# drapado/PINGS

Hardware: AMD Instinct MI355X
Metric: raster fwd+bwd Mpix/s @1M Gaussians 1080p (higher is better)
Workload: dtype f32; 1 GPU; surfel rasteriser fwd+bwd, 1000000 Gaussians, 1920x1080, one view per GPU; gaussians=1000000, width=1920, height=1080

## Files before the change

include/pings_hip.h:

```cpp
#ifndef PINGS_HIP_H_
#define PINGS_HIP_H_

#include <stddef.h>
#include <stdint.h>

#if defined(__cplusplus)
#define PINGS_EXTERN_C extern "C"
#else
#define PINGS_EXTERN_C
#endif
#define PINGS_API PINGS_EXTERN_C __attribute__((visibility("default")))

#define PINGS_OK 0
#define PINGS_ERR_ARG 1
#define PINGS_ERR_HIP 2
#define PINGS_ERR_CAPACITY 3


#define PINGS_ABI_VERSION 11
PINGS_API int pings_abi_version(void);
PINGS_API const char* pings_last_error(void);

PINGS_API int pings_prof_enable(int on);
PINGS_API int pings_prof_only(const char* stage);
// ... 69 lines not shown

PINGS_API int pings_raster_backward(const pings_raster_settings* s, int P, int64_t num_instances,
                                    const float* means3D, const float* colors,
                                    const float* opacities, const float* scales,
                                    const float* rotations, const void* geom_blob,
                                    const void* binning_blob, const void* image_blob,
                                    const float* out_color, const float* out_normal,
                                    const float* out_depth, const float* out_alpha,
                                    const float* dL_dcolor, const float* dL_dnormal,
                                    const float* dL_ddepth, const float* dL_dalpha,
                                    void* bwd_blob, float* dL_dmeans3D, float* dL_dmeans2D,
                                    float* dL_dcolors, float* dL_dopacities, float* dL_dscales,
                                    float* dL_drotations, float* dL_dtau, int footprint_class,
                                    void* stream);

PINGS_API int pings_raster_debug_lists(const void* binning_blob, int64_t num_instances,
                                       int image_height, int image_width, uint32_t* point_list,
                                       uint32_t* ranges_xy, void* stream);
PINGS_API int pings_raster_debug_image(const void* image_blob, int image_height, int image_width,
                                       float* final_T, uint32_t* n_contrib, void* stream);
PINGS_API int pings_raster_debug_occlusion(const void* geom_blob, int P, int image_height, int image_width,
                                           uint32_t* occ_bucket, uint16_t* occ_bsat, int32_t* occ_nb,
                                           void* stream);


PINGS_API size_t pings_raster2d_geom_bytes(int P, int image_height, int image_width);
PINGS_API size_t pings_raster2d_binning_bytes(int64_t num_instances, int image_height, int image_width);
PINGS_API size_t pings_raster2d_image_bytes(int image_height, int image_width);

PINGS_API int pings_raster2d_preprocess(const pings_raster_settings* s, int P, const float* means3D,
                                        const float* colors, const float* opacities, const float* scales,
                                        const float* rotations, void* geom_blob, int32_t* radii,
                                        const int32_t* live_rows_dev, int dyn_rows, const int32_t* const* aux_dev,
                                        int aux_words, int32_t* aux_host, int64_t* num_instances, void* stream);

PINGS_API int pings_raster2d_render(const pings_raster_settings* s, int P, int64_t num_instances, void* geom_blob,
                                    void* binning_blob, void* image_blob, float* out_color, float* out_allmap,
                                    void* stream);

PINGS_API size_t pings_raster2d_backward_bytes(int P, int64_t num_instances);

PINGS_API int pings_raster2d_backward(const pings_raster_settings* s, int P, int64_t num_instances,
                                      const float* scales, const float* rotations, const void* geom_blob,
                                      const void* binning_blob, const void* image_blob, const float* dL_dcolor,
                                      const float* dL_dallmap, void* bwd_blob, float* dL_dmeans3D,
                                      float* dL_dmeans2D, float* dL_dcolors, float* dL_dopacities,
// ... 714 lines not shown
```

pings_amd/_abi.py:

```python
from __future__ import annotations

import ctypes as C

ABI_VERSION = 11

RASTER_SURFEL, RASTER_3DGS, RASTER_2DGS = 0, 1, 2
HEAD_COLOR, HEAD_SEMANTIC = 0, 1
REG_SINGULAR, REG_ILL_CONDITIONED, REG_NONFINITE = 1, 2, 4
REG_F_NORMALS, REG_F_DIV_GRAD, REG_F_WEIGHTED = 1, 2, 4
REG_COLOR_PHOTO, REG_COLOR_CONSIST = 1, 2
MC_ALLOW_DEGENERATE, MC_ASCENT = 1, 2
ADAMW_MAX_JOBS, ADAMW_CHUNK = 48, 4096
EVAL_VIEW_RECORD, EVAL_PAIR_RECORD = 9, 12
EVAL_EXTENT = 1
LOOP_MAX_R, LOOP_MAX_S, LOOP_MAX_D = 32, 128, 16
LOOP_MAX_Q, LOOP_MAX_C = 16, 65536
LIDAR_MAX_CAMS, LIDAR_MAX_LIDARS = 8, 8
TSDF_BLOCK = 8
TSDF_EXTENT, TSDF_TABLE_FULL = 1, 2

vp = C.c_void_p
i32, i64, f32, f64, sz = C.c_int, C.c_int64, C.c_float, C.c_double, C.c_size_t


# ... 152 lines not shown
    "pings_prof_report": (i32, [C.c_char_p, sz]),
    "pings_ssim_partials_count": (sz, [i32, i32, i32]),
    "pings_ssim_forward": (i32, [vp, vp, i32, i32, i32, i32, vp, vp, vp, vp, vp, vp]),
    "pings_ssim_backward": (i32, [vp, vp, i32, i32, i32, vp, vp, vp, vp, vp, vp]),
    "pings_raster_mark_visible": (i32, [vp, i32, C.POINTER(RasterSettings), vp, vp]),
    "pings_raster_geom_bytes": (sz, [i32, i32, i32]),
    "pings_raster_binning_bytes": (sz, [i64, i32, i32]),
    "pings_raster_image_bytes": (sz, [i32, i32]),
    "pings_raster_preprocess": (i32, [C.POINTER(RasterSettings), i32, vp, vp, vp, vp, vp, vp, vp, C.POINTER(i64),
                                      C.POINTER(i32), vp]),
    "pings_raster_preprocess_dyn": (i32, [C.POINTER(RasterSettings), i32, vp, vp, vp, vp, vp, vp, vp, vp, i32,
                                          C.POINTER(vp), i32, C.POINTER(i32), C.POINTER(i64), C.POINTER(i32), vp]),
    "pings_raster_render": (i32, [C.POINTER(RasterSettings), i32, i64, vp, vp, vp, vp, vp, vp, vp, vp, i32, vp]),
    "pings_raster_tile_sort_bytes": (sz, [i64, C.POINTER(i32)]),
    "pings_raster_tile_sort": (i32, [vp, i64, i32, i32, vp, vp, vp, i32, vp]),
    "pings_raster_scan_bytes": (sz, [i64]),
    "pings_raster_scan_u32": (i32, [vp, i64, i32, i32, vp, vp, sz, vp]),
    "pings_raster_backward_bytes": (sz, [i32, i64]),
    "pings_raster_backward": (i32, [C.POINTER(RasterSettings), i32, i64, vp, vp, vp, vp, vp, vp, vp, vp, vp, vp, vp, vp,
                                    vp, vp, vp, vp, vp, vp, vp, vp, vp, vp, vp, vp, i32, vp]),
    "pings_raster_debug_lists": (i32, [vp, i64, i32, i32, vp, vp, vp]),
    "pings_raster_debug_image": (i32, [vp, i32, i32, vp, vp, vp]),
    "pings_raster_debug_occlusion": (i32, [vp, i32, i32, i32, vp, vp, C.POINTER(C.c_int32), vp]),
    "pings_raster2d_geom_bytes": (sz, [i32, i32, i32]),
    "pings_raster2d_binning_bytes": (sz, [i64, i32, i32]),
    "pings_raster2d_image_bytes": (sz, [i32, i32]),
    "pings_raster2d_preprocess": (i32, [C.POINTER(RasterSettings), i32, vp, vp, vp, vp, vp, vp, vp, vp, i32,
                                        C.POINTER(vp), i32, C.POINTER(i32), C.POINTER(i64), vp]),
    "pings_raster2d_render": (i32, [C.POINTER(RasterSettings), i32, i64, vp, vp, vp, vp, vp, vp]),
    "pings_raster2d_backward_bytes": (sz, [i32, i64]),
    "pings_raster2d_backward": (i32, [C.POINTER(RasterSettings), i32, i64, vp, vp, vp, vp, vp, vp, vp, vp, vp, vp, vp,
                                      vp, vp, vp, vp]),
    "pings_raster2d_debug_lists": (i32, [vp, i64, i32, i32, vp, vp, vp]),
    "pings_raster2d_debug_image": (i32, [vp, i32, i32, vp, vp, vp, vp]),
    "pings_knn_compact_entries": (sz, [i64]),
    "pings_knn_compact_build": (i32, [vp, i64, vp, sz, vp]),
    "pings_knn_blocks_entries": (sz, [i64]),
    "pings_knn_blocks_build": (i32, [C.POINTER(KnnMap), i64, i64, i32, vp, sz, vp, vp, vp]),
    "pings_knn_search": (i32, [C.POINTER(KnnMap), vp, i64, vp, vp, vp, vp, vp]),
    "pings_knn_cells": (i32, [C.POINTER(KnnMap), vp, i64, i64, vp, vp, vp]),
    "pings_query_feature_forward": (i32, [C.POINTER(KnnMap), C.POINTER(QfTables), vp, i64, vp, vp, vp, vp, vp, vp, vp,
                                          vp, vp, vp, vp, vp]),
    "pings_query_feature_accumulate": (i32, [vp, vp, i64, vp, vp]),
    "pings_query_feature_scratch_bytes": (sz, [i64, i32, i64]),
    "pings_query_feature_backward": (i32, [C.POINTER(QfTables), vp, vp, i64, i32, vp, vp, vp, vp, vp, vp, i64, vp, vp,
                                           vp, vp, vp]),
# ... 163 lines not shown
```

pings_amd/csrc/raster_blend_fwd.hip:

```cpp
#include "raster_common.hpp"

namespace pings {
namespace raster {

template <int MODE>
__device__ __forceinline__ void blend_fwd_wave_body(
    const KParams& p, const uint2* __restrict__ ranges, const uint32_t* __restrict__ point_list,
    const float4* __restrict__ rec, const uint32_t* __restrict__ gval, float* __restrict__ out_color,
    float* __restrict__ out_normal, float* __restrict__ out_depth, float* __restrict__ out_alpha,
    float* __restrict__ final_T, uint32_t* __restrict__ n_contrib, float* __restrict__ inst_wq,
    uint32_t* __restrict__ inst_cntq, const uint32_t* __restrict__ tile_order,
    const uint32_t* __restrict__ seg_tile_unit0, const unsigned block) {
  __shared__ float4 sA_[4][64], sB_[4][64], sC_[4][64], sD_[4][64];
  __shared__ uint32_t sSlot_[4][64];
  __shared__ int sE_[4][64];
  __shared__ float sW_[4][64];
  __shared__ uint32_t sCnt_[4][64];

  const int lane = threadIdx.x & 63, q = (int)(threadIdx.x >> 6);
  float4 *sA = sA_[q], *sB = sB_[q], *sC = sC_[q], *sD = sD_[q];
  uint32_t *sSlot = sSlot_[q], *sCnt = sCnt_[q];
  int* sE = sE_[q];
  float* sW = sW_[q];
  const int tile = (int)tile_order[block];
// ... 754 lines not shown
  if (MODE == MODE_3DGS) {
    const uint4 c = cq[i];
    inst_cnt[i] = c.x + c.y + c.z + c.w;
  }
}

__device__ inline uint32_t wave_reduce_sum_u32(uint32_t v) {
#pragma unroll
  for (int off = 32; off > 0; off >>= 1) v += (uint32_t)__shfl_xor((int)v, off, 64);
  return v;
}

constexpr int SMALL_RUN = 16;
template <typename T>
__global__ __launch_bounds__(256) void per_gaussian_sum_kernel(
    int P, const uint32_t* __restrict__ gidx_sorted, const uint32_t* __restrict__ nvalid,
    const uint32_t* __restrict__ offsets_sorted, const uint32_t* __restrict__ tiles_sorted,
    const T* __restrict__ inst, T* __restrict__ out) {
  const int r = strided_rank(P);
  const int lane = threadIdx.x & 63;
  uint32_t n = 0, base = 0;
  if (r >= 0 && (uint32_t)r < *nvalid) {
    n = tiles_sorted[r];
    base = offsets_sorted[r] - n;
  }
  T sum = (T)0;
  if (n <= (uint32_t)SMALL_RUN)
    for (uint32_t k = 0; k < n; ++k) sum += inst[base + k];
  unsigned long long m = __ballot(n > (uint32_t)SMALL_RUN);
  while (m) {
    const int src = __ffsll((long long)m) - 1;
    m &= m - 1;
    const uint32_t nb = lane_value(n, src);
    const uint32_t bb = lane_value(base, src);
    T acc = (T)0, acc1 = (T)0, acc2 = (T)0, acc3 = (T)0;
    uint32_t k = lane;
    for (; k + 192 < nb; k += 256) {
      acc += inst[bb + k];
      acc1 += inst[bb + k + 64];
      acc2 += inst[bb + k + 128];
      acc3 += inst[bb + k + 192];
    }
    for (; k < nb; k += 64) acc += inst[bb + k];
    acc = (acc + acc1) + (acc2 + acc3);
    if constexpr (sizeof(T) == 4 && !std::is_integral<T>::value) {
      acc = wave_sum_to_all(acc);
    } else {
      acc = (T)wave_reduce_sum_u32((uint32_t)acc);
    }
    if (lane == src) sum = acc;
  }
  if (r >= 0) out[gidx_sorted[r]] = sum;
}

struct FwdOut {
  float *color, *normal, *depth, *alpha;
};

template <int MODE>
static int launch_blend_fwd_wave(const KParams& kp, const BlendPlan& plan, int64_t I, int num_tiles, const GeomState& gs,
                          const BinState& bs, const ImageState& im, const FwdOut& o, hipStream_t st) {
  const uint32_t seg = plan.seg;
  if (I > 0) PINGS_HIP_CHECK(hipMemsetAsync(bs.inst_wq, 0, 16 * (size_t)I, st));
  if (I > 0 && MODE == MODE_3DGS) PINGS_HIP_CHECK(hipMemsetAsync(bs.inst_cntq, 0, 16 * (size_t)I, st));
  if (!plan.seg_on) {
    hipLaunchKernelGGL((blend_fwd_wave_kernel<MODE>), dim3(num_tiles), dim3(256), 0, st, kp, bs.ranges,
                       bs.point_list, gs.rec, bs.gval, o.color, o.normal, o.depth, o.alpha,
                       im.final_T, im.n_contrib, bs.inst_wq, bs.inst_cntq, bs.tile_order,
                       (const uint32_t*)nullptr);
  } else {
    hipLaunchKernelGGL(seg_plan_kernel, dim3(1), dim3(1024), 0, st, bs.ranges, num_tiles, 2u * seg, seg,
                       bs.seg_max_units, bs.seg_head, bs.seg_unit_tile, bs.seg_unit_seg, bs.seg_tile_unit0);
    PINGS_LAUNCH_CHECK();
    const dim3 gseg(bs.seg_max_units);
    uint16_t* const rel = plan.seg_reuse ? bs.seg_rel : nullptr;
// ... 72 lines not shown
```

pings_amd/csrc/raster_common.hpp:

```cpp
#pragma once
#include <cstdlib>
#include <type_traits>

#include "common.hpp"

namespace pings {
namespace raster {

constexpr int TILE = 16;
constexpr int BLOCK = TILE * TILE;
constexpr float NEAR_Z = 0.2f;
constexpr float LOWPASS = 0.3f;
constexpr float ALPHA_MAX = 0.99f;
constexpr float ALPHA_MIN = 1.0f / 255.0f;
constexpr float T_EPS = 1e-4f;
constexpr float DEPTH_ALPHA_EPS = 1e-10f;
constexpr float DEN_EPS = 1e-6f;
constexpr uint32_t CULLED_KEY = 0xFFFFFFFFu;
constexpr int DS_NB = 1 << 20;
constexpr uint32_t DS_LIMIT = 4096u;
constexpr int DS_SHARDS = 64;
constexpr int DS_KMIN = 2 * DS_SHARDS, DS_SHIFT = DS_KMIN + 1, DS_FLAG = DS_KMIN + 2, DS_HEAD = DS_KMIN + 8;
constexpr float OCC_THR = 9.5f;
constexpr float OCC_FIX = 4096.f;
constexpr uint16_t OCC_ALL = 0xFFFFu;

constexpr int MODE_SURFEL = 0;
constexpr int MODE_3DGS = 1;
constexpr int RECT_TIGHT = 0, RECT_3SIGMA = 1, RECT_ELLIPSE = 2;

constexpr int GRAD_ROW = 16;
constexpr int CH = 64;
enum GradSlot {
  G_MX = 0, G_MY = 1, G_CONX = 2, G_CONY = 3, G_CONZ = 4, G_OPAC = 5,
  G_R = 6, G_G = 7, G_B = 8, G_NX = 9, G_NY = 10, G_NZ = 11, G_Q = 12, G_PZ = 13,
  G_ZLO = 14, G_ZHI = 15
};

struct FrameSummary {
  uint32_t overflow, pad0;
  unsigned long long stats[3];
  int32_t aux[8];
  uint32_t seq;
  uint32_t pad;
};
// ... 165 lines not shown
int tile_sort_library(const KeyT* keys_in, int64_t n, int bits, KeyT* keys_out, uint32_t* vals_out, void* temp,
                      size_t temp_bytes, hipStream_t st);

int launch_blend_fwd(int mode, const KParams& kp, const BlendPlan& plan, int P, int64_t I, const GeomState& gs,
                     const BinState& bs, const ImageState& im, float* out_color, float* out_normal, float* out_depth,
                     float* out_alpha, void* per_gaussian, hipStream_t st);

__device__ inline int lane_value(int v, int src) { return __builtin_amdgcn_readlane(v, src); }
__device__ inline uint32_t lane_value(uint32_t v, int src) { return (uint32_t)__builtin_amdgcn_readlane((int)v, src); }
__device__ inline float lane_value(float v, int src) {
  return __builtin_bit_cast(float, __builtin_amdgcn_readlane(__builtin_bit_cast(int, v), src));
}

__device__ inline int dealt_rank(int num_waves, int wave, int lane) {
  return lane < 16 ? lane * num_waves + wave : ((lane >> 4) * num_waves + wave) * 16 + (lane & 15);
}
__device__ inline int strided_rank(int P) {
  const int num_waves = (int)(gridDim.x * (blockDim.x >> 6));
  const int wave = (int)(blockIdx.x * (blockDim.x >> 6) + (threadIdx.x >> 6));
  const int r = dealt_rank(num_waves, wave, (int)(threadIdx.x & 63));
  return r < P ? r : -1;
}

typedef float f2 __attribute__((ext_vector_type(2)));
__device__ inline f2 f2s(float x) { return f2{x, x}; }
__device__ inline f2 fma2(f2 a, f2 b, f2 c) { return __builtin_elementwise_fma(a, b, c); }
__device__ inline f2 sel2(bool c0, bool c1, f2 a, f2 b) { return f2{c0 ? a.x : b.x, c1 ? a.y : b.y}; }

typedef unsigned long long lmask;
struct cmask {
  unsigned long long bits;
};
enum { LM_OGT = 2, LM_OGE = 3, LM_OLT = 4, LM_OLE = 5 };
__device__ inline cmask mask_lt(float a, float b) { return cmask{__builtin_amdgcn_fcmpf(a, b, LM_OLT)}; }
__device__ inline cmask mask_le(float a, float b) { return cmask{__builtin_amdgcn_fcmpf(a, b, LM_OLE)}; }
__device__ inline cmask mask_gt(float a, float b) { return cmask{__builtin_amdgcn_fcmpf(a, b, LM_OGT)}; }
__device__ inline cmask mask_ge(float a, float b) { return cmask{__builtin_amdgcn_fcmpf(a, b, LM_OGE)}; }
__device__ inline lmask operator&(cmask a, cmask b) { return a.bits & b.bits; }
__device__ inline lmask operator&(lmask a, cmask b) { return a & b.bits; }
__device__ inline lmask operator&(cmask a, lmask b) { return a.bits & b; }
__device__ inline lmask operator|(cmask a, cmask b) { return a.bits | b.bits; }
__device__ inline lmask operator~(cmask a) { return ~a.bits; }
__device__ inline int mask_count(lmask m) { return __builtin_popcountll(m); }
__device__ inline float mask_sel(lmask m, float a, float b) {
  float r;
  asm("v_cndmask_b32_e64 %0, %1, %2, %3" : "=v"(r) : "v"(b), "v"(a), "s"(m));
// ... 293 lines not shown
```

pings_amd/csrc/raster_fwd.hip:

```cpp
#include <hipcub/hipcub.hpp>

#include <algorithm>
#include <chrono>
#include <type_traits>

#include "raster_common.hpp"

namespace pings {
namespace raster {

__device__ inline void to_camera(const float* __restrict__ V, float x, float y, float z, float& px,
                                 float& py, float& pz) {
  px = ((V[0] * x + V[4] * y) + V[8] * z) + V[12];
  py = ((V[1] * x + V[5] * y) + V[9] * z) + V[13];
  pz = ((V[2] * x + V[6] * y) + V[10] * z) + V[14];
}

__global__ __launch_bounds__(256) void mark_visible_kernel(const float* __restrict__ pos, int N,
                                                            const float* __restrict__ V,
                                                            const float* __restrict__ Pm,
                                                            uint8_t* __restrict__ present, int depth_only) {
  const int i = blockIdx.x * blockDim.x + threadIdx.x;
  if (i >= N) return;
  float px, py, pz;
  to_camera(V, pos[3 * i], pos[3 * i + 1], pos[3 * i + 2], px, py, pz);
  const float hx = ((Pm[0] * px + Pm[4] * py) + Pm[8] * pz) + Pm[12];
  const float hy = ((Pm[1] * px + Pm[5] * py) + Pm[9] * pz) + Pm[13];
  const float hw = ((Pm[3] * px + Pm[7] * py) + Pm[11] * pz) + Pm[15];
  const float pw = 1.0f / (hw + 1e-7f);
  const float nx = hx * pw, ny = hy * pw;
  present[i] = (pz > NEAR_Z) && (depth_only || ((nx >= -1.3f) && (nx <= 1.3f) && (ny >= -1.3f) && (ny <= 1.3f)));
}

template <int MODE>
__device__ inline uint32_t preprocess_gaussian(
    const KParams& p, int g, const float* __restrict__ means3D, const float* __restrict__ colors,
    const float* __restrict__ opacities, const float* __restrict__ scales,
    const float* __restrict__ rotations, float4* __restrict__ rec, uint4* __restrict__ rect,
    uint32_t* __restrict__ depth_key, uint32_t* __restrict__ gidx, int32_t* __restrict__ radii) {
  const float* V = p.view;
  const float* Pm = p.proj_raw;

  gidx[g] = (uint32_t)g;
  uint32_t key = CULLED_KEY;
  uint4 rc = make_uint4(0u, 0u, 0u, 0u);
  int rad = 0;

  float px, py, pz;
  to_camera(V, means3D[3 * g], means3D[3 * g + 1], means3D[3 * g + 2], px, py, pz);
  bool ok = pz > NEAR_Z;
  if (p.live && g < p.dyn_rows && g >= *p.live) ok = false;

  const float hx = ((Pm[0] * px + Pm[4] * py) + Pm[8] * pz) + Pm[12];
  const float hy = ((Pm[1] * px + Pm[5] * py) + Pm[9] * pz) + Pm[13];
  const float hw = ((Pm[3] * px + Pm[7] * py) + Pm[11] * pz) + Pm[15];
  const float pw = 1.0f / (hw + 1e-7f);
  const float ndx = hx * pw, ndy = hy * pw;
  const float mx = ((ndx + 1.0f) * (float)p.W - 1.0f) * 0.5f;
  const float my = ((ndy + 1.0f) * (float)p.H - 1.0f) * 0.5f;

  const float qr = rotations[4 * g], qx = rotations[4 * g + 1], qy = rotations[4 * g + 2],
              qz = rotations[4 * g + 3];
// ... 95 lines not shown
        const float thr_u = 2.0f * logf(opac / p.occ_amin);
        const float lam_min = mid - sqrtf(fmaxf(mid * mid - det, 0.0f));
        uint32_t inner = 0xFFFFFFFFu;
        if (thr_u * lam_min >= 50.0f) {
          const float exu = sqrtf(thr_u * cxx), eyu = sqrtf(thr_u * cyy);
          const int ix0 = max(xmin, (int)ceilf((mx - exu) / (float)TILE - 0.02f));
          const int ix1 = min(xmax, (int)floorf((mx + exu - 15.0f) / (float)TILE + 0.02f) + 1);
          const int iy0 = max(ymin, (int)ceilf((my - eyu) / (float)TILE - 0.02f));
          const int iy1 = min(ymax, (int)floorf((my + eyu - 15.0f) / (float)TILE + 0.02f) + 1);
          if (ix1 > ix0 && iy1 > iy0)
            inner = (uint32_t)min(ix0 - xmin, 255) | ((uint32_t)min(xmax - ix1, 255) << 8) |
                    ((uint32_t)min(iy0 - ymin, 255) << 16) | ((uint32_t)min(ymax - iy1, 255) << 24);
        }
        const uint32_t covers = inner;
        rc = make_uint4(covers, (uint32_t)xmin | ((uint32_t)ymin << 16),
                        (uint32_t)xmax | ((uint32_t)ymax << 16), (uint32_t)tiles);
        rad = (int)radius;
      }
    }
  }
  depth_key[g] = key;
  rect[g] = rc;
  radii[g] = rad;
  if (key != CULLED_KEY) {
    rec[4 * g + 0] = make_float4(mx, my, opac, pz);
    rec[4 * g + 1] = make_float4(conic_x, conic_y, conic_z, rz);
    rec[4 * g + 2] = make_float4(colors[3 * g], colors[3 * g + 1], colors[3 * g + 2], q);
    rec[4 * g + 3] = make_float4(nx, ny, nz, 0.0f);
  }
  return key;
}

template <int MODE>
__global__ __launch_bounds__(256) void preprocess_kernel(
    KParams p, const float* __restrict__ means3D, const float* __restrict__ colors,
    const float* __restrict__ opacities, const float* __restrict__ scales,
    const float* __restrict__ rotations, float4* __restrict__ rec, uint4* __restrict__ rect,
    uint32_t* __restrict__ depth_key, uint32_t* __restrict__ gidx, int32_t* __restrict__ radii,
    uint32_t* __restrict__ ds_head) {
  __shared__ uint32_t sm[8];
  const int g = blockIdx.x * blockDim.x + threadIdx.x;
  uint32_t key = CULLED_KEY;
  if (g < p.P)
    key = preprocess_gaussian<MODE>(p, g, means3D, colors, opacities, scales, rotations, rec, rect, depth_key, gidx, radii);
  if (!ds_head) return;
  uint32_t mx = key != CULLED_KEY ? key : 0u, mn = key != CULLED_KEY ? ~key : 0u;
#pragma unroll
  for (int o = 32; o > 0; o >>= 1) {
    mx = max(mx, (uint32_t)__shfl_xor((int)mx, o, 64));
    mn = max(mn, (uint32_t)__shfl_xor((int)mn, o, 64));
  }
  const int wave = threadIdx.x >> 6;
  if ((threadIdx.x & 63) == 0) { sm[wave] = mx; sm[4 + wave] = mn; }
  __syncthreads();
  if (threadIdx.x == 0) {
    mx = max(max(sm[0], sm[1]), max(sm[2], sm[3]));
    mn = max(max(sm[4], sm[5]), max(sm[6], sm[7]));
    if (mx | mn) {
      atomicMax(&ds_head[blockIdx.x % DS_SHARDS], mx);
      atomicMax(&ds_head[DS_SHARDS + blockIdx.x % DS_SHARDS], mn);
    }
  }
}

constexpr int SMALL_RECT = 8;
constexpr int STAT_SHARDS = 256;

struct RectLane {
  uint32_t g, n;
  int xmin, ymin, wdt, hgt;
};
template <typename Serial, typename CoopBegin, typename Coop>
__device__ inline void walk_rects(const RectLane& me, int gx, Serial serial, CoopBegin coop_begin, Coop coop) {
  const int lane = threadIdx.x & 63;
  if (me.n != 0u && me.n <= (uint32_t)SMALL_RECT) {
    int x = 0, y = 0;
    for (uint32_t k = 0; k < me.n; ++k) {
      serial(me.xmin + x, me.ymin + y);
      if (++x == me.wdt) { x = 0; ++y; }
    }
  }
  unsigned long long m = __ballot(me.n > (uint32_t)SMALL_RECT);
  while (m) {
    const int src = __ffsll((long long)m) - 1;
    m &= m - 1;
    const uint32_t n = lane_value(me.n, src);
    const int x0 = lane_value(me.xmin, src), y0 = lane_value(me.ymin, src), wdt = lane_value(me.wdt, src);
    const float inv_w = 1.0f / (float)wdt;
    coop_begin(src);
// ... 247 lines not shown
                                                           uint32_t* __restrict__ rank_of) {
  const int r = blockIdx.x * 256 + threadIdx.x;
  if (r < P) rank_of[gidx_sorted[r]] = (uint32_t)r;
}

__global__ __launch_bounds__(64) void count_valid_kernel(int P, const uint32_t* __restrict__ depth_key_sorted,
                                                         uint32_t* __restrict__ nvalid) {
  const int lane = threadIdx.x;
  long long lo = 0, hi = P;
  while (lo < hi) {
    const long long span = hi - lo;
    const long long step = (span + 63) / 64;
    const long long pos = lo + (long long)lane * step;
    const bool valid = pos < hi && depth_key_sorted[pos] < CULLED_KEY;
    const int nv = __popcll(__ballot(valid));
    if (nv == 0) { hi = lo; break; }
    const long long last_valid = lo + (long long)(nv - 1) * step;
    lo = last_valid + 1;
    hi = min(hi, last_valid + step);
  }
  if (lane == 0) *nvalid = (uint32_t)lo;
}

__device__ inline uint32_t rank_bucket(int r, int nb, uint32_t nvalid) {
  if (r < 0 || nvalid == 0u) return 0u;
  const uint32_t b = (uint32_t)(((unsigned long long)r * (unsigned long long)nb) / (unsigned long long)nvalid);
  return min(b, (uint32_t)nb - 1u);
}

template <bool DENSE>
__global__ __launch_bounds__(256) void occl_budget_kernel(int P, int gx, int nb,
                                                          const uint32_t* __restrict__ gidx_sorted,
                                                          const uint4* __restrict__ rect,
                                                          const float4* __restrict__ rec,
                                                          const uint32_t* __restrict__ nvalid, int num_tiles,
                                                          uint32_t* __restrict__ bucket) {
  const int r = strided_rank(P);
  const uint32_t nv = *nvalid;
  RectLane me = rect_lane(r, gidx_sorted, rect, nv);
  if (me.n != 0u) {
    const uint4 rc = rect[me.g];
    const int x0 = me.xmin + (int)(rc.x & 255u), x1 = (int)(rc.z & 0xFFFF) - (int)((rc.x >> 8) & 255u);
    const int y0 = me.ymin + (int)((rc.x >> 16) & 255u), y1 = (int)(rc.z >> 16) - (int)(rc.x >> 24);
    if (x1 > x0 && y1 > y0) {
      me.xmin = x0; me.ymin = y0; me.wdt = x1 - x0; me.hgt = y1 - y0; me.n = (uint32_t)((x1 - x0) * (y1 - y0));
    } else {
      me.n = 0u;
    }
  }
  float4 ra = make_float4(0.f, 0.f, 0.f, 0.f), rb = ra;
  if (me.n != 0u) {
// ... 103 lines not shown
  __syncthreads();
  const uint32_t sat = tile < num_tiles ? sSat[t] : 0u;
  if (g == 0) {
    uint32_t m = min(sat, (uint32_t)nb - 1u);
#pragma unroll
    for (int o = 32; o > 0; o >>= 1) m = max(m, (uint32_t)__shfl_xor((int)m, o, 64));
    if (t == 0) atomicMax(bmax, m);
  }
  unsigned long long word = 0ull;
  for (int u = 0; u < per; ++u) {
    const unsigned long long w = __ballot(tile < num_tiles && (uint32_t)(g * per + u) <= sat);
    if (t == u) word = w;
  }
  if (t < per) mask[(size_t)(g * per + t) * gridDim.x + blockIdx.x] = word;
}

__global__ __launch_bounds__(256) void count_kept_kernel(int P, int gx, int nb, int words,
                                                         const uint32_t* __restrict__ gidx_sorted,
                                                         const uint4* __restrict__ rect,
                                                         const unsigned long long* __restrict__ mask,
                                                         const uint32_t* __restrict__ nvalid,
                                                         const uint32_t* __restrict__ bmax,
                                                         uint32_t* __restrict__ tiles_sorted,
                                                         unsigned long long* __restrict__ pairs_full) {
  const int r = strided_rank(P);
  const int lane = threadIdx.x & 63;
  const uint32_t nv = *nvalid;
  const RectLane me = rect_lane(r, gidx_sorted, rect, nv);
  const uint32_t bk = rank_bucket(r, nb, nv);
  const uint32_t items = bk <= *bmax ? rect_items(me) : 0u;
  uint32_t kept = 0, acc = 0;
  if (items != 0u && items <= (uint32_t)SMALL_ITEMS)
    walk_items_serial(me, items, gx, mask + (size_t)bk * words,
                      [&](int, unsigned long long bits) { kept += (uint32_t)__popcll(bits); });
  int cur = -1;
  auto flush = [&]() {
    if (cur < 0) return;
#pragma unroll
    for (int off = 32; off > 0; off >>= 1) acc += (uint32_t)__shfl_xor((int)acc, off, 64);
    if (lane == cur) kept = acc;
  };
  walk_items_coop(
      __ballot(items > (uint32_t)SMALL_ITEMS), me, items, gx, bk, mask, words,
      [&](int src) { flush(); cur = src; acc = 0; },
      [&](int, unsigned long long bits) { acc += (uint32_t)__popcll(bits); });
  flush();
  if (r >= 0) tiles_sorted[r] = kept;
  uint32_t tot = me.n;
#pragma unroll
  for (int off = 32; off > 0; off >>= 1) tot += (uint32_t)__shfl_xor((int)tot, off, 64);
  const unsigned long long vis = __ballot(me.n != 0u);
  uint32_t kept_w = r >= 0 ? kept : 0u;
#pragma unroll
  for (int off = 32; off > 0; off >>= 1) kept_w += (uint32_t)__shfl_xor((int)kept_w, off, 64);
  if (lane == 0 && tot) {
    const int shard = (int)((blockIdx.x * (blockDim.x >> 6) + (threadIdx.x >> 6)) & (STAT_SHARDS - 1));
    atomicAdd(pairs_full + 3 * shard, (unsigned long long)tot);
    atomicAdd(pairs_full + 3 * shard + 1, (unsigned long long)__popcll(vis));
    atomicAdd(pairs_full + 3 * shard + 2, (unsigned long long)kept_w);
  }
}

template <typename KeyT>
__global__ __launch_bounds__(256) void duplicate_kernel(int P, int gx, int nb, int words,
                                                         const uint32_t* __restrict__ gidx_sorted,
                                                         const uint32_t* __restrict__ offsets_sorted,
                                                         const uint32_t* __restrict__ tiles_sorted,
                                                         const uint4* __restrict__ rect,
                                                         const unsigned long long* __restrict__ mask,
                                                         const uint32_t* __restrict__ nvalid,
                                                         KeyT* __restrict__ tile_key,
                                                         uint32_t* __restrict__ gval) {
  const int r = strided_rank(P);
  const int lane = threadIdx.x & 63;
  const uint32_t nv = *nvalid;
  const RectLane me = rect_lane(r, gidx_sorted, rect, nv);
  const uint32_t bk = rank_bucket(r, nb, nv);
  const uint32_t kept = r >= 0 ? tiles_sorted[r] : 0u;
  uint32_t o = r >= 0 ? offsets_sorted[r] - kept : 0u;
  const uint32_t items = kept != 0u ? rect_items(me) : 0u;
  const bool coop = items > (uint32_t)SMALL_ITEMS || kept > SMALL_KEPT;
  if (items != 0u && !coop)
    walk_items_serial(me, items, gx, mask + (size_t)bk * words, [&](int s, unsigned long long bits) {
      while (bits) {
        tile_key[o] = (KeyT)(s + __builtin_ctzll(bits));
        gval[o] = me.g;
        ++o;
        bits &= bits - 1;
      }
    });
  uint32_t so = 0, sg = 0;
  walk_items_coop(
      __ballot(items != 0u && coop), me, items, gx, bk, mask, words,
      [&](int src) {
        so = lane_value(o, src);
        sg = lane_value(me.g, src);
      },
      [&](int s, unsigned long long bits) {
        unsigned long long todo = __ballot(bits != 0ull);
        while (todo) {
          const int j = __ffsll((long long)todo) - 1;
          todo &= todo - 1;
          const uint32_t blo = lane_value((uint32_t)bits, j), bhi = lane_value((uint32_t)(bits >> 32), j);
// ... 24 lines not shown
  return PINGS_OK;
}

template <typename KeyT>
__global__ __launch_bounds__(256) void tile_ranges_kernel(int64_t I, const KeyT* __restrict__ key,
                                                           uint2* __restrict__ ranges) {
  const int64_t i = (int64_t)blockIdx.x * blockDim.x + threadIdx.x;
  if (i >= I) return;
  const uint32_t t = (uint32_t)key[i];
  if (i == 0 || key[i - 1] != t) ranges[t].x = (uint32_t)i;
  if (i == I - 1 || key[i + 1] != t) ranges[t].y = (uint32_t)(i + 1);
}

struct AuxPtrs {
  const int32_t* p[8];
};
__global__ __launch_bounds__(64) void frame_summary_kernel(const uint32_t* __restrict__ overflow,
                                                           const unsigned long long* __restrict__ shards, AuxPtrs aux,
                                                           int aux_words, FrameSummary* __restrict__ out, uint32_t seq) {
  __shared__ unsigned long long part[3][64];
  const int lane = threadIdx.x;
  unsigned long long a0 = 0, a1 = 0, a2 = 0;
  for (int i = lane; i < STAT_SHARDS; i += 64) {
    a0 += shards[3 * i]; a1 += shards[3 * i + 1]; a2 += shards[3 * i + 2];
  }
  part[0][lane] = a0; part[1][lane] = a1; part[2][lane] = a2;
  __syncthreads();
  if (lane < 3) {
    unsigned long long t = 0;
    for (int i = 0; i < 64; ++i) t += part[lane][i];
    out->stats[lane] = t;
  }
  if (lane == 4) out->overflow = overflow ? *overflow : 0u;
  if (lane >= 8 && lane < 16) out->aux[lane - 8] = (lane - 8 < aux_words && aux.p[lane - 8]) ? *aux.p[lane - 8] : 0;
  __threadfence_system();
  __syncthreads();
  if (lane == 0) __hip_atomic_store(&out->seq, seq, __ATOMIC_RELEASE, __HIP_MEMORY_SCOPE_SYSTEM);
}

static int make_params(const pings_raster_settings* s, int P, const RasterKnobs& knobs, KParams& kp) {
  if (int e = fill_camera(s, P, kp)) return e;
  kp.occ_amin = knobs.occ_amin;
  kp.rect_rule = knobs.rect_rule;
  kp.live = nullptr;
  kp.dyn_rows = 0;
  return PINGS_OK;
}

static int tile_bits(int num_tiles) {
  int b = 1;
  while ((1 << b) < num_tiles) ++b;
  return b;
}

}
}

using namespace pings::raster;

PINGS_API int pings_raster_mark_visible(const float* positions, int N,
                                        const pings_raster_settings* s, uint8_t* present,
                                        void* stream) {
  PINGS_ARG_CHECK(s && s->viewmatrix && s->projmatrix_raw, "null settings / matrices");
  if (N == 0) return PINGS_OK;
  PINGS_ARG_CHECK(N > 0 && positions && present, "null pointer");
  const int depth_only = read_knobs().mark_depth_only;
  hipLaunchKernelGGL(mark_visible_kernel, dim3(pings::ceil_div(N, 256)), dim3(256), 0,
                     pings::as_stream(stream), positions, N, s->viewmatrix, s->projmatrix_raw,
                     present, depth_only);
  PINGS_LAUNCH_CHECK();
  return PINGS_OK;
}

PINGS_API int pings_raster_preprocess(const pings_raster_settings* s, int P, const float* means3D,
                                      const float* colors, const float* opacities,
                                      const float* scales, const float* rotations,
                                      void* geom_blob, int32_t* radii, int64_t* num_instances,
                                      int32_t* footprint_class, void* stream) {
  return pings_raster_preprocess_dyn(s, P, means3D, colors, opacities, scales, rotations, geom_blob, radii, nullptr, 0,
                                     nullptr, 0, nullptr, num_instances, footprint_class, stream);
}

PINGS_API int pings_raster_preprocess_dyn(const pings_raster_settings* s, int P, const float* means3D,
                                          const float* colors, const float* opacities, const float* scales,
                                          const float* rotations, void* geom_blob, int32_t* radii,
                                          const int32_t* live_rows_dev, int dyn_rows,
                                          const int32_t* const* aux_dev, int aux_words, int32_t* aux_host,
                                          int64_t* num_instances, int32_t* footprint_class, void* stream) {
  const RasterKnobs knobs = read_knobs();
  KParams kp;
  if (int e = make_params(s, P, knobs, kp)) return e;
  PINGS_ARG_CHECK(num_instances != nullptr && footprint_class != nullptr, "null output");
  *num_instances = 0;
  *footprint_class = 1;
  PINGS_ARG_CHECK(aux_words >= 0 && aux_words <= 8 && (aux_words == 0 || (aux_dev && aux_host)), "0..8 aux words");
  PINGS_ARG_CHECK(!live_rows_dev || (dyn_rows >= 0 && dyn_rows <= P), "dyn_rows must lie in 0..P");
  PINGS_ARG_CHECK(P > 0 || aux_words == 0, "aux words need a non-empty frame");
  if (P == 0) return PINGS_OK;
  kp.live = live_rows_dev;
  kp.dyn_rows = live_rows_dev ? dyn_rows : 0;
  PINGS_ARG_CHECK(P > 0 && means3D && colors && opacities && scales && rotations && geom_blob && radii,
                  "null pointer");
  hipStream_t st = pings::as_stream(stream);
  const int num_tiles = kp.gx * kp.gy;
  GeomState gs = carve_geom(geom_blob, P, num_tiles);
  const dim3 grid(pings::ceil_div(P, 256)), block(256);
  const bool occlusion = knobs.occlusion;
  bool library_sort = knobs.library_sort;
  PINGS_HIP_CHECK(hipMemsetAsync(gs.zero_begin, 0, gs.zero_bytes, st));
  {
    pings::prof::Scope ps("preprocess", st);
    with_mode(s->mode, [&](auto m) {
      hipLaunchKernelGGL(preprocess_kernel<m()>, grid, block, 0, st, kp, means3D, colors,
                         opacities, scales, rotations, gs.rec, gs.rect, gs.depth_key, gs.gidx, radii,
                         library_sort ? (uint32_t*)nullptr : gs.ds_head);
    });
    PINGS_LAUNCH_CHECK();
  }
  static thread_local FrameSummary* host_sum = nullptr;
  static thread_local FrameSummary* host_sum_dev = nullptr;
  static thread_local uint32_t frame_seq = 0;
  if (!host_sum) {
    PINGS_HIP_CHECK(hipHostMalloc(reinterpret_cast<void**>(&host_sum), sizeof(FrameSummary), hipHostMallocMapped | hipHostMallocPortable));
    PINGS_HIP_CHECK(hipHostGetDevicePointer(reinterpret_cast<void**>(&host_sum_dev), host_sum, 0));
    host_sum->seq = 0;
  }
  AuxPtrs aux;
  for (int i = 0; i < 8; ++i) aux.p[i] = i < aux_words ? aux_dev[i] : nullptr;
  for (int attempt = 0;; ++attempt) {
    size_t tb = gs.temp_bytes;
    if (library_sort) {
      pings::prof::Scope ps("depth_sort", st);
      PINGS_HIP_CHECK(hipcub::DeviceRadixSort::SortPairs(gs.temp, tb, gs.depth_key, gs.depth_key_sorted,
                                                         gs.gidx, gs.gidx_sorted, P, 0, 32, st));
      hipLaunchKernelGGL(count_valid_kernel, dim3(1), dim3(64), 0, st, P, gs.depth_key_sorted, gs.nvalid);
      PINGS_LAUNCH_CHECK();
      hipLaunchKernelGGL(invert_perm_kernel, grid, block, 0, st, P, gs.gidx_sorted, gs.rank_of);
      PINGS_LAUNCH_CHECK();
// ... 6 lines not shown
        return e;
      hipLaunchKernelGGL(ds_scatter_kernel, grid, block, 0, st, P, gs.depth_key, gs.ds_head, gs.ds_off, gs.rank_of,
                         gs.depth_key_sorted, gs.ds_idx, gs.gidx_sorted);
      PINGS_LAUNCH_CHECK();
      hipLaunchKernelGGL(ds_rank_kernel, grid, block, 0, st, gs.depth_key_sorted, gs.ds_idx, gs.ds_head, gs.ds_off,
                         gs.gidx_sorted, gs.rank_of, gs.nvalid);
      PINGS_LAUNCH_CHECK();
    }
    if (occlusion) {
      {
        pings::prof::Scope ps("occl_setup", st);
        if (attempt > 0)
          PINGS_HIP_CHECK(hipMemsetAsync(gs.occ_bucket, 0, sizeof(uint32_t) * (size_t)num_tiles * gs.occ_nb, st));
      }
      {
        pings::prof::Scope ps("occl_budget", st);
        hipLaunchKernelGGL(knobs.occ_walk_lanes ? occl_budget_kernel<false> : occl_budget_kernel<true>, grid, block, 0,
                           st, P, kp.gx, gs.occ_nb, gs.gidx_sorted, gs.rect, gs.rec, gs.nvalid, num_tiles, gs.occ_bucket);
        PINGS_LAUNCH_CHECK();
      }
    }
    {
      pings::prof::Scope ps("occl_scan", st);
      if (attempt > 0) PINGS_HIP_CHECK(hipMemsetAsync(gs.stats, 0, (3 * STAT_SHARDS + 1) * sizeof(unsigned long long), st));
      hipLaunchKernelGGL(occl_scan_kernel, dim3(gs.occ_words), dim3(512), 0, st, num_tiles, gs.occ_nb, gs.occ_bucket,
                         gs.occ_bsat, gs.occ_mask, gs.occ_bmax);
      PINGS_LAUNCH_CHECK();
    }
    {
      pings::prof::Scope ps("tile_count_scan", st);
      hipLaunchKernelGGL(count_kept_kernel, grid, block, 0, st, P, kp.gx, gs.occ_nb, gs.occ_words, gs.gidx_sorted,
                         gs.rect, gs.occ_mask, gs.nvalid, gs.occ_bmax, gs.tiles_sorted, gs.stats);
      PINGS_LAUNCH_CHECK();
    }
    const uint32_t seq = ++frame_seq ? frame_seq : ++frame_seq;
    hipLaunchKernelGGL(frame_summary_kernel, dim3(1), dim3(64), 0, st,
                       library_sort ? (const uint32_t*)nullptr : gs.ds_head + DS_FLAG, gs.stats, aux, aux_words,
                       host_sum_dev, seq);
    PINGS_LAUNCH_CHECK();
    {
      pings::prof::Scope ps("tile_count_scan", st);
      if (int e = raster_scan_u32(gs.tiles_sorted, P, true, gs.offsets_sorted, gs.temp, gs.temp_bytes, knobs.library_scan, st))
        return e;
    }
    {
      const auto t_start = std::chrono::steady_clock::now();
      unsigned spins = 0;
// ... 33 lines not shown
  PINGS_ARG_CHECK(s->mode == PINGS_RASTER_3DGS || out_normal, "surfel mode needs out_normal");
  PINGS_ARG_CHECK(I >= 0 && I < (int64_t)0x7FFFFFFF, "instance count out of range");
  PINGS_ARG_CHECK(P == 0 || (geom_blob && per_gaussian), "null pointer");
  hipStream_t st = pings::as_stream(stream);
  const int num_tiles = kp.gx * kp.gy;
  GeomState gs = carve_geom(geom_blob, P, num_tiles);
  BinState bs = carve_binning(binning_blob, I, num_tiles, knobs.blend_seg);
  ImageState im = carve_image(image_blob, kp.W, kp.H);

  {
    const char* z0 = reinterpret_cast<const char*>(bs.ranges);
    const char* z1 = I > 0 ? (s->mode == PINGS_RASTER_3DGS ? reinterpret_cast<const char*>(bs.inst_cnt + I)
                                                             : reinterpret_cast<const char*>(bs.inst_qmask + I + 1))
                           : reinterpret_cast<const char*>(bs.ranges + num_tiles);
    PINGS_HIP_CHECK(hipMemsetAsync(bs.ranges, 0, pings::align_up((size_t)(z1 - z0)), st));
  }
  if (I > 0) {
    auto bin = [&](auto* key, auto* key_sorted) -> int {
      using KeyT = std::remove_pointer_t<decltype(key)>;
      {
        pings::prof::Scope ps("duplicate", st);
        hipLaunchKernelGGL(duplicate_kernel<KeyT>, dim3(pings::ceil_div(P, 256)), dim3(256), 0, st, P,
                           kp.gx, gs.occ_nb, gs.occ_words, gs.gidx_sorted, gs.offsets_sorted, gs.tiles_sorted,
                           gs.rect, gs.occ_mask, gs.nvalid, key, bs.gval);
        PINGS_LAUNCH_CHECK();
      }
      const int bits = tile_bits(num_tiles);
      const KeyT* sorted = key_sorted;
      {
        pings::prof::Scope ps("tile_sort", st);
        if (knobs.library_tile_sort || bits > 16) {
          if (int e = tile_sort_library<KeyT>(key, I, bits, key_sorted, bs.point_list, bs.temp, bs.temp_bytes, st)) return e;
        } else {
          if (bits > 8) sorted = key;
          if (int e = tile_sort<KeyT>(key, I, bits, key_sorted, bs.slot_val, bits > 8 ? key : key_sorted, bs.point_list,
                                      reinterpret_cast<uint32_t*>(bs.temp), st))
            return e;
        }
      }
      {
        pings::prof::Scope ps("tile_ranges", st);
        hipLaunchKernelGGL(tile_ranges_kernel<KeyT>, dim3((unsigned)pings::ceil_div<int64_t>(I, 256)), dim3(256), 0,
                           st, I, sorted, bs.ranges);
        PINGS_LAUNCH_CHECK();
      }
      return PINGS_OK;
    };
// ... 14 lines not shown
```

pings_amd/csrc/raster_layout.hip:

```cpp
#include <hipcub/hipcub.hpp>

#include <algorithm>
#include <cmath>
#include <cstdlib>
#include <cstring>

#include "raster_common.hpp"

namespace pings {
namespace raster {

static size_t sort_temp_bytes(int64_t n) {
  size_t a = 0, b = 0;
  (void)hipcub::DeviceRadixSort::SortPairs(nullptr, a, (uint32_t*)nullptr, (uint32_t*)nullptr,
                                     (uint32_t*)nullptr, (uint32_t*)nullptr, (int)n, 0, 32);
  (void)hipcub::DeviceScan::InclusiveSum(nullptr, b, (uint32_t*)nullptr, (uint32_t*)nullptr,
                                         (int)std::max<int64_t>(n, DS_NB + n / 256 + 2));
  size_t c = 0;
  (void)hipcub::DeviceRadixSort::SortPairs(nullptr, c, (uint16_t*)nullptr, (uint16_t*)nullptr,
                                           (uint32_t*)nullptr, (uint32_t*)nullptr, (int)n, 0, 16);
  if (c > a) a = c;
  a = std::max(a, std::max(tile_sort_library_bytes(n), tile_sort_table_bytes(n)));
  a = std::max(a, raster_scan_bytes(std::max<int64_t>(n, DS_NB + n / 256 + 2)));
  return align_up(a > b ? a : b) + 256;
// ... 1 lines not shown

int occlusion_buckets(int num_tiles) {
  int nb = 256;
  while (nb > 32 && (size_t)nb * (size_t)num_tiles > ((size_t)1 << 21)) nb >>= 1;
  return nb;
}

GeomState carve_geom(void* blob, int P, int num_tiles) {
  Carver c(blob);
  GeomState g;
  const size_t n = (size_t)(P > 0 ? P : 1);
  const size_t nt = (size_t)(num_tiles > 0 ? num_tiles : 1);
  g.rec = c.take<float4>(4 * n);
  g.rect = c.take<uint4>(n);
  g.depth_key = c.take<uint32_t>(n);
  g.depth_key_sorted = c.take<uint32_t>(n);
  g.gidx = c.take<uint32_t>(n);
  g.gidx_sorted = c.take<uint32_t>(n);
  g.rank_of = c.take<uint32_t>(n);
  g.tiles_sorted = c.take<uint32_t>(n);
  g.offsets_sorted = c.take<uint32_t>(n);
  g.occ_nb = occlusion_buckets((int)nt);
  g.occ_bucket = c.take<uint32_t>(nt * (size_t)g.occ_nb);
  g.stats = c.take<unsigned long long>(3 * 256 + 1);
  g.occ_bmax = g.stats ? reinterpret_cast<uint32_t*>(g.stats + 3 * 256) : nullptr;
  const size_t nblk = (n + 255) / 256;
  g.ds_words = DS_HEAD + (size_t)DS_NB + nblk;
  g.ds_head = c.take<uint32_t>(g.ds_words);
  g.ds_cnt = g.ds_head ? g.ds_head + DS_HEAD : nullptr;
  g.zero_begin = reinterpret_cast<char*>(g.occ_bucket);
  g.zero_bytes = g.ds_head ? align_up((size_t)(reinterpret_cast<char*>(g.ds_head + g.ds_words) - g.zero_begin)) : 0;
  g.occ_bsat = c.take<uint16_t>(nt);
  g.occ_words = (int)((nt + 63) / 64);
  g.occ_mask = c.take<unsigned long long>((size_t)g.occ_nb * (size_t)g.occ_words + 1);
  g.nvalid = c.take<uint32_t>(1);
  g.ds_off = c.take<uint32_t>((size_t)DS_NB + nblk + 1);
  g.ds_idx = c.take<uint32_t>(n);
  g.summary = c.take<FrameSummary>(1);
  g.temp_bytes = sort_temp_bytes((int64_t)n);
  g.temp = c.take<char>(g.temp_bytes);
  g.total = c.total();
  return g;
}

BinState carve_binning(void* blob, int64_t I, int num_tiles, uint32_t seg) {
  Carver c(blob);
  BinState b;
  const size_t n = (size_t)(I > 0 ? I : 1);
// ... 170 lines not shown
```

Measured before the change: 2615 Mpix/s.

## Move pair/visibility stats to preprocess, skip culled ranks, use log-spaced front rank buckets

Pair and visible-count statistics now accumulate in the preprocess kernel, not the occlusion count kernel. A retry therefore clears only the kept-count shards, and the stat layout becomes named constants. The count, duplicate and per-tile reduction kernels skip rect and offset loads and output writes for ranks with no kept tiles. The duplicate kernel also zeroes the per-gaussian buffer inline, which removes a separate clear. The rank-to-bucket mapping gives front depth ranks finer, logarithmically spaced occlusion buckets, which changes culling granularity. A host helper exposes that mapping.

```diff
diff --git a/include/pings_hip.h b/include/pings_hip.h
--- a/include/pings_hip.h
+++ b/include/pings_hip.h
@@ -115,6 +115,8 @@
 PINGS_API int pings_raster_debug_occlusion(const void* geom_blob, int P, int image_height, int image_width,
                                            uint32_t* occ_bucket, uint16_t* occ_bsat, int32_t* occ_nb,
                                            void* stream);
+PINGS_API int pings_raster_rank_bucket(const int32_t* ranks, int64_t n, int occ_nb, uint32_t nvalid,
+                                       uint32_t* buckets);
 
 
 PINGS_API size_t pings_raster2d_geom_bytes(int P, int image_height, int image_width);
diff --git a/pings_amd/_abi.py b/pings_amd/_abi.py
--- a/pings_amd/_abi.py
+++ b/pings_amd/_abi.py
@@ -198,6 +198,7 @@
     "pings_raster_debug_lists": (i32, [vp, i64, i32, i32, vp, vp, vp]),
     "pings_raster_debug_image": (i32, [vp, i32, i32, vp, vp, vp]),
     "pings_raster_debug_occlusion": (i32, [vp, i32, i32, i32, vp, vp, C.POINTER(C.c_int32), vp]),
+    "pings_raster_rank_bucket": (i32, [vp, i64, i32, C.c_uint32, vp]),
     "pings_raster2d_geom_bytes": (sz, [i32, i32, i32]),
     "pings_raster2d_binning_bytes": (sz, [i64, i32, i32]),
     "pings_raster2d_image_bytes": (sz, [i32, i32]),
diff --git a/pings_amd/csrc/raster_blend_fwd.hip b/pings_amd/csrc/raster_blend_fwd.hip
--- a/pings_amd/csrc/raster_blend_fwd.hip
+++ b/pings_amd/csrc/raster_blend_fwd.hip
@@ -800,7 +800,7 @@
   uint32_t n = 0, base = 0;
   if (r >= 0 && (uint32_t)r < *nvalid) {
     n = tiles_sorted[r];
-    base = offsets_sorted[r] - n;
+    if (n != 0u) base = offsets_sorted[r] - n;
   }
   T sum = (T)0;
   if (n <= (uint32_t)SMALL_RUN)
@@ -828,7 +828,7 @@
     }
     if (lane == src) sum = acc;
   }
-  if (r >= 0) out[gidx_sorted[r]] = sum;
+  if (n != 0u) out[gidx_sorted[r]] = sum;
 }
 
 struct FwdOut {
diff --git a/pings_amd/csrc/raster_common.hpp b/pings_amd/csrc/raster_common.hpp
--- a/pings_amd/csrc/raster_common.hpp
+++ b/pings_amd/csrc/raster_common.hpp
@@ -21,6 +21,10 @@
 constexpr uint32_t DS_LIMIT = 4096u;
 constexpr int DS_SHARDS = 64;
 constexpr int DS_KMIN = 2 * DS_SHARDS, DS_SHIFT = DS_KMIN + 1, DS_FLAG = DS_KMIN + 2, DS_HEAD = DS_KMIN + 8;
+constexpr int STAT_SHARDS = 256;
+constexpr int STAT_PAIRS = 0, STAT_VISIBLE = STAT_SHARDS, STAT_KEPT = 2 * STAT_SHARDS;
+constexpr int STAT_BMAX = 3 * STAT_SHARDS, STAT_WORDS = STAT_BMAX + 1, STAT_RETRY_WORDS = STAT_WORDS - STAT_KEPT;
+static_assert((STAT_SHARDS & (STAT_SHARDS - 1)) == 0, "the shard of a wave is its number modulo a power of two");
 constexpr float OCC_THR = 9.5f;
 constexpr float OCC_FIX = 4096.f;
 constexpr uint16_t OCC_ALL = 0xFFFFu;
@@ -232,6 +236,30 @@
   return r < P ? r : -1;
 }
 
+constexpr int RB_LW = 4, RB_LS = 4;
+__host__ __device__ inline uint32_t rank_bucket_log2(uint32_t x) { return 31u - (uint32_t)__builtin_clz(x); }
+__host__ __device__ inline uint32_t rank_bucket(int r, int nb, uint32_t nvalid) {
+  if (r < 0 || nvalid == 0u) return 0u;
+  const uint32_t ur = (uint32_t)r, unb = (uint32_t)nb;
+  if (ur >= nvalid) return unb - 1u;
+  const uint32_t eq = (nvalid - 1u) / unb + 1u;
+  uint32_t J = 0u;
+  if ((eq >> RB_LW) != 0u) {
+    J = rank_bucket_log2(eq >> RB_LW) + 2u;
+    if (J > (unb >> (RB_LS + 1))) J = unb >> (RB_LS + 1);
+  }
+  const uint32_t front_ranks = J ? 1u << (RB_LW + RB_LS + J - 1u) : 0u, front_buckets = J << RB_LS;
+  if (ur < front_ranks) {
+    const uint32_t q = ur >> RB_LW;
+    if ((q >> RB_LS) == 0u) return q;
+    const uint32_t k = rank_bucket_log2(q) - RB_LS;
+    return (k << RB_LS) + (q >> k);
+  }
+  const uint32_t b = front_buckets + (uint32_t)(((unsigned long long)(ur - front_ranks) * (unb - front_buckets)) /
+                                                (unsigned long long)(nvalid - front_ranks));
+  return b < unb ? b : unb - 1u;
+}
+
 typedef float f2 __attribute__((ext_vector_type(2)));
 __device__ inline f2 f2s(float x) { return f2{x, x}; }
 __device__ inline f2 fma2(f2 a, f2 b, f2 c) { return __builtin_elementwise_fma(a, b, c); }
diff --git a/pings_amd/csrc/raster_fwd.hip b/pings_amd/csrc/raster_fwd.hip
--- a/pings_amd/csrc/raster_fwd.hip
+++ b/pings_amd/csrc/raster_fwd.hip
@@ -37,7 +37,8 @@
     const KParams& p, int g, const float* __restrict__ means3D, const float* __restrict__ colors,
     const float* __restrict__ opacities, const float* __restrict__ scales,
     const float* __restrict__ rotations, float4* __restrict__ rec, uint4* __restrict__ rect,
-    uint32_t* __restrict__ depth_key, uint32_t* __restrict__ gidx, int32_t* __restrict__ radii) {
+    uint32_t* __restrict__ depth_key, uint32_t* __restrict__ gidx, int32_t* __restrict__ radii,
+    uint32_t& tiles_out) {
   const float* V = p.view;
   const float* Pm = p.proj_raw;
 
@@ -179,6 +180,7 @@
   depth_key[g] = key;
   rect[g] = rc;
   radii[g] = rad;
+  tiles_out = rc.w;
   if (key != CULLED_KEY) {
     rec[4 * g + 0] = make_float4(mx, my, opac, pz);
     rec[4 * g + 1] = make_float4(conic_x, conic_y, conic_z, rz);
@@ -186,6 +188,10 @@
     rec[4 * g + 3] = make_float4(nx, ny, nz, 0.0f);
   }
   return key;
+}
+
+__device__ inline int stat_shard() {
+  return (int)((blockIdx.x * (blockDim.x >> 6) + (threadIdx.x >> 6)) & (STAT_SHARDS - 1));
 }
 
 template <int MODE>
@@ -194,12 +200,24 @@
     const float* __restrict__ opacities, const float* __restrict__ scales,
     const float* __restrict__ rotations, float4* __restrict__ rec, uint4* __restrict__ rect,
     uint32_t* __restrict__ depth_key, uint32_t* __restrict__ gidx, int32_t* __restrict__ radii,
-    uint32_t* __restrict__ ds_head) {
+    uint32_t* __restrict__ ds_head, unsigned long long* __restrict__ stats) {
   __shared__ uint32_t sm[8];
   const int g = blockIdx.x * blockDim.x + threadIdx.x;
-  uint32_t key = CULLED_KEY;
+  uint32_t key = CULLED_KEY, tiles = 0u;
   if (g < p.P)
-    key = preprocess_gaussian<MODE>(p, g, means3D, colors, opacities, scales, rotations, rec, rect, depth_key, gidx, radii);
+    key = preprocess_gaussian<MODE>(p, g, means3D, colors, opacities, scales, rotations, rec, rect, depth_key, gidx, radii,
+                                    tiles);
+  {
+    const unsigned long long vis = __ballot(tiles != 0u);
+    uint32_t tot = tiles;
+#pragma unroll
+    for (int o = 32; o > 0; o >>= 1) tot += (uint32_t)__shfl_xor((int)tot, o, 64);
+    if ((threadIdx.x & 63) == 0 && tot) {
+      const int shard = stat_shard();
+      atomicAdd(stats + STAT_PAIRS + shard, (unsigned long long)tot);
+      atomicAdd(stats + STAT_VISIBLE + shard, (unsigned long long)__popcll(vis));
+    }
+  }
   if (!ds_head) return;
   uint32_t mx = key != CULLED_KEY ? key : 0u, mn = key != CULLED_KEY ? ~key : 0u;
 #pragma unroll
@@ -221,7 +239,6 @@
 }
 
 constexpr int SMALL_RECT = 8;
-constexpr int STAT_SHARDS = 256;
 
 struct RectLane {
   uint32_t g, n;
@@ -515,11 +532,6 @@
   if (lane == 0) *nvalid = (uint32_t)lo;
 }
 
-__device__ inline uint32_t rank_bucket(int r, int nb, uint32_t nvalid) {
-  if (r < 0 || nvalid == 0u) return 0u;
-  const uint32_t b = (uint32_t)(((unsigned long long)r * (unsigned long long)nb) / (unsigned long long)nvalid);
-  return min(b, (uint32_t)nb - 1u);
-}
 
 template <bool DENSE>
 __global__ __launch_bounds__(256) void occl_budget_kernel(int P, int gx, int nb,
@@ -669,13 +681,13 @@
                                                          const uint32_t* __restrict__ nvalid,
                                                          const uint32_t* __restrict__ bmax,
                                                          uint32_t* __restrict__ tiles_sorted,
-                                                         unsigned long long* __restrict__ pairs_full) {
+                                                         unsigned long long* __restrict__ stats) {
   const int r = strided_rank(P);
   const int lane = threadIdx.x & 63;
   const uint32_t nv = *nvalid;
-  const RectLane me = rect_lane(r, gidx_sorted, rect, nv);
   const uint32_t bk = rank_bucket(r, nb, nv);
-  const uint32_t items = bk <= *bmax ? rect_items(me) : 0u;
+  const RectLane me = rect_lane(bk <= *bmax ? r : -1, gidx_sorted, rect, nv);
+  const uint32_t items = rect_items(me);
   uint32_t kept = 0, acc = 0;
   if (items != 0u && items <= (uint32_t)SMALL_ITEMS)
     walk_items_serial(me, items, gx, mask + (size_t)bk * words,
@@ -693,19 +705,10 @@
       [&](int, unsigned long long bits) { acc += (uint32_t)__popcll(bits); });
   flush();
   if (r >= 0) tiles_sorted[r] = kept;
-  uint32_t tot = me.n;
-#pragma unroll
-  for (int off = 32; off > 0; off >>= 1) tot += (uint32_t)__shfl_xor((int)tot, off, 64);
-  const unsigned long long vis = __ballot(me.n != 0u);
   uint32_t kept_w = r >= 0 ? kept : 0u;
 #pragma unroll
   for (int off = 32; off > 0; off >>= 1) kept_w += (uint32_t)__shfl_xor((int)kept_w, off, 64);
-  if (lane == 0 && tot) {
-    const int shard = (int)((blockIdx.x * (blockDim.x >> 6) + (threadIdx.x >> 6)) & (STAT_SHARDS - 1));
-    atomicAdd(pairs_full + 3 * shard, (unsigned long long)tot);
-    atomicAdd(pairs_full + 3 * shard + 1, (unsigned long long)__popcll(vis));
-    atomicAdd(pairs_full + 3 * shard + 2, (unsigned long long)kept_w);
-  }
+  if (lane == 0 && kept_w) atomicAdd(stats + STAT_KEPT + stat_shard(), (unsigned long long)kept_w);
 }
 
 template <typename KeyT>
@@ -717,15 +720,18 @@
                                                          const unsigned long long* __restrict__ mask,
                                                          const uint32_t* __restrict__ nvalid,
                                                          KeyT* __restrict__ tile_key,
-                                                         uint32_t* __restrict__ gval) {
+                                                         uint32_t* __restrict__ gval,
+                                                         uint32_t* __restrict__ per_gaussian) {
+  const int i = blockIdx.x * blockDim.x + threadIdx.x;
+  if (i < P) per_gaussian[i] = 0u;
   const int r = strided_rank(P);
   const int lane = threadIdx.x & 63;
+  const uint32_t kept = r >= 0 ? tiles_sorted[r] : 0u;
   const uint32_t nv = *nvalid;
-  const RectLane me = rect_lane(r, gidx_sorted, rect, nv);
-  const uint32_t bk = rank_bucket(r, nb, nv);
-  const uint32_t kept = r >= 0 ? tiles_sorted[r] : 0u;
-  uint32_t o = r >= 0 ? offsets_sorted[r] - kept : 0u;
-  const uint32_t items = kept != 0u ? rect_items(me) : 0u;
+  const RectLane me = rect_lane(kept != 0u ? r : -1, gidx_sorted, rect, nv);
+  const uint32_t bk = kept != 0u ? rank_bucket(r, nb, nv) : 0u;
+  uint32_t o = kept != 0u ? offsets_sorted[r] - kept : 0u;
+  const uint32_t items = rect_items(me);
   const bool coop = items > (uint32_t)SMALL_ITEMS || kept > SMALL_KEPT;
   if (items != 0u && !coop)
     walk_items_serial(me, items, gx, mask + (size_t)bk * words, [&](int s, unsigned long long bits) {
@@ -796,7 +802,7 @@
   const int lane = threadIdx.x;
   unsigned long long a0 = 0, a1 = 0, a2 = 0;
   for (int i = lane; i < STAT_SHARDS; i += 64) {
-    a0 += shards[3 * i]; a1 += shards[3 * i + 1]; a2 += shards[3 * i + 2];
+    a0 += shards[STAT_PAIRS + i]; a1 += shards[STAT_VISIBLE + i]; a2 += shards[STAT_KEPT + i];
   }
   part[0][lane] = a0; part[1][lane] = a1; part[2][lane] = a2;
   __syncthreads();
@@ -843,6 +849,13 @@
                      pings::as_stream(stream), positions, N, s->viewmatrix, s->projmatrix_raw,
                      present, depth_only);
   PINGS_LAUNCH_CHECK();
+  return PINGS_OK;
+}
+
+PINGS_API int pings_raster_rank_bucket(const int32_t* ranks, int64_t n, int occ_nb, uint32_t nvalid,
+                                       uint32_t* buckets) {
+  PINGS_ARG_CHECK(n >= 0 && occ_nb > 0 && (n == 0 || (ranks && buckets)), "null pointer / non-positive bucket count");
+  for (int64_t i = 0; i < n; ++i) buckets[i] = rank_bucket(ranks[i], occ_nb, nvalid);
   return PINGS_OK;
 }
 
@@ -887,7 +900,7 @@
     with_mode(s->mode, [&](auto m) {
       hipLaunchKernelGGL(preprocess_kernel<m()>, grid, block, 0, st, kp, means3D, colors,
                          opacities, scales, rotations, gs.rec, gs.rect, gs.depth_key, gs.gidx, radii,
-                         library_sort ? (uint32_t*)nullptr : gs.ds_head);
+                         library_sort ? (uint32_t*)nullptr : gs.ds_head, gs.stats);
     });
     PINGS_LAUNCH_CHECK();
   }
@@ -940,7 +953,8 @@
     }
     {
       pings::prof::Scope ps("occl_scan", st);
-      if (attempt > 0) PINGS_HIP_CHECK(hipMemsetAsync(gs.stats, 0, (3 * STAT_SHARDS + 1) * sizeof(unsigned long long), st));
+      if (attempt > 0)
+        PINGS_HIP_CHECK(hipMemsetAsync(gs.stats + STAT_KEPT, 0, STAT_RETRY_WORDS * sizeof(unsigned long long), st));
       hipLaunchKernelGGL(occl_scan_kernel, dim3(gs.occ_words), dim3(512), 0, st, num_tiles, gs.occ_nb, gs.occ_bucket,
                          gs.occ_bsat, gs.occ_mask, gs.occ_bmax);
       PINGS_LAUNCH_CHECK();
@@ -1020,7 +1034,7 @@
         pings::prof::Scope ps("duplicate", st);
         hipLaunchKernelGGL(duplicate_kernel<KeyT>, dim3(pings::ceil_div(P, 256)), dim3(256), 0, st, P,
                            kp.gx, gs.occ_nb, gs.occ_words, gs.gidx_sorted, gs.offsets_sorted, gs.tiles_sorted,
-                           gs.rect, gs.occ_mask, gs.nvalid, key, bs.gval);
+                           gs.rect, gs.occ_mask, gs.nvalid, key, bs.gval, reinterpret_cast<uint32_t*>(per_gaussian));
         PINGS_LAUNCH_CHECK();
       }
       const int bits = tile_bits(num_tiles);
diff --git a/pings_amd/csrc/raster_layout.hip b/pings_amd/csrc/raster_layout.hip
--- a/pings_amd/csrc/raster_layout.hip
+++ b/pings_amd/csrc/raster_layout.hip
@@ -47,8 +47,8 @@
   g.offsets_sorted = c.take<uint32_t>(n);
   g.occ_nb = occlusion_buckets((int)nt);
   g.occ_bucket = c.take<uint32_t>(nt * (size_t)g.occ_nb);
-  g.stats = c.take<unsigned long long>(3 * 256 + 1);
-  g.occ_bmax = g.stats ? reinterpret_cast<uint32_t*>(g.stats + 3 * 256) : nullptr;
+  g.stats = c.take<unsigned long long>(STAT_WORDS);
+  g.occ_bmax = g.stats ? reinterpret_cast<uint32_t*>(g.stats + STAT_BMAX) : nullptr;
   const size_t nblk = (n + 255) / 256;
   g.ds_words = DS_HEAD + (size_t)DS_NB + nblk;
   g.ds_head = c.take<uint32_t>(g.ds_words);
```

After: 2740 Mpix/s (median of 6 runs). 4.8% higher.
